# mhauskn/dqn-hfo

Hardware: AMD Instinct MI355X
Metric: DQN updates/sec, 1v0 HFO, 4x1024 MLP, minibatch 256 (higher is better)
Workload: dtype f32

## Files before the change

dqn-hfo_amd/capi.py:

```python
import ctypes as C
import os

from ._build import LIB, build

MAX_HIDDEN = 8
NSTEP_MAX = 64
DP_ID_BYTES = 128
DP_PER_LAYER, DP_HALF_GRADS, DP_SHARD_OPT = 1, 2, 4
DP_UNVERIFIED_OK = 256
TUNE_FP16_WGRAD_PER_LAYER = 1
TUNE_SEPARATE_HEAD_SEED = 2
TUNE_BWD_UNSHIFTED = 4
TUNE_SEPARATE_ACTOR_HEAD_BWD = 8
TUNE_SEPARATE_Q_TRAIN = 16
TUNE_SEPARATE_FIRST_LAYER = 32
TUNE_SEPARATE_CRITIC_FIRST_LAYERS = 64
TUNE_LATE_GATHER = 128
TUNE_NO_KERNARG_PRELOAD = 256
PLAN_FORMS = ("fp16", "data_parallel", "bwd_shifted_critic", "bwd_shifted_actor", "head_wgrad_rides_critic", "head_wgrad_rides_actor",
              "q_train_in_dgrad", "head_seed_fused", "dqda_head_bwd", "critic_l0_rides", "first_layers_merged", "early_gather_l0", "dp_tails_ride", "prioritized", "n_step", "target_smoothing")
LOSS_SCALE_STATIC, LOSS_SCALE_DYNAMIC = 0, 1
FP32, FP16 = 0, 1
ACTOR, CRITIC, ACTOR_TARGET, CRITIC_TARGET = 0, 1, 2, 3
KIND_W, KIND_M, KIND_V, KIND_G = 0, 1, 2, 3
SOLVERS = ("Adam", "SGD", "Nesterov", "AdaGrad", "RMSProp", "AdaDelta")


LR_POLICIES = ("fixed", "step", "exp", "inv", "multistep", "poly", "sigmoid")
LR_MAX_STEPVALUES = 16
REGULARIZATIONS = ("L2", "L1")


class Config(C.Structure):
# ... 282 lines not shown
```

dqn-hfo_amd/csrc/gemm_bodies.hip.h:

```cpp
#pragma once
#include <hip/hip_runtime.h>

#include <cstdint>

#include "learner_args.hip.h"

namespace dqnhip {


__host__ __device__ __forceinline__ void tile_of_counts(int tiles_p, int tiles_q, int b, int& tile_p, int& tile_q) {
  const bool xmap = (tiles_p & 7) == 0;
  const int j = xmap ? b >> 3 : b;
  const int d = j / tiles_q;
  tile_q = j - d * tiles_q;
  tile_p = xmap ? d * 8 + (b & 7) : d;
}
constexpr int kTileDecodeMaxQ = 1024, kTileDecodeMaxTiles = 1 << 18;
__host__ __device__ __forceinline__ uint32_t tile_magic(int tiles_q) { return (uint32_t)((0x80000000ull + (uint32_t)tiles_q - 1) / (uint32_t)tiles_q); }
__host__ __device__ __forceinline__ bool tile_magic_covers(int tiles_p, int tiles_q) {
  return tiles_p >= 1 && tiles_q >= 1 && tiles_q <= kTileDecodeMaxQ && (int64_t)tiles_p * tiles_q <= kTileDecodeMaxTiles;
}
__host__ __device__ __forceinline__ void tile_decode(int tiles_p, int tiles_q, uint32_t magic, int b, int& tile_p, int& tile_q) {
  const bool xmap = (tiles_p & 7) == 0;
  const int j = xmap ? b >> 3 : b;
// ... 476 lines not shown
  __syncthreads();
  f32x4 v = f32x4{0.f, 0.f, 0.f, 0.f};
  if (wave == 0) v = reduce_accumulator<1>(smem, 0, lane);
  return v;
}
__device__ __forceinline__ void dgrad_narrow_body(const GemmProblem& pr, int tile_p, int tile_q, float* smem) {
  const f32x4 v = dgrad_narrow_tile<4>(pr, tile_p, tile_q, smem);
  if ((threadIdx.x >> 6) == 0) {
    const int lane = threadIdx.x & 63, li = lane & 15, lg = lane >> 4;
    const int q = tile_q * 16 + li, p = tile_p * 16 + (lg << 2);
    *reinterpret_cast<f32x4*>(pr.C + (size_t)q * pr.ldc + p) = v;
  }
}

constexpr int kWgradRing = 4;
template <int TPB, int TQB>
__device__ __forceinline__ void wgrad_direct_body(const GemmProblem& pr, int tile_p, int tile_q, float* smem) {
  constexpr int NACC = TPB * 4 * TQB * 4;
  const int lane = threadIdx.x & 63, wave = threadIdx.x >> 6;
  const int li = lane & 15, lg = lane >> 4;
  const int p0 = tile_p * 64 * TPB, q0 = tile_q * 64 * TQB;
  const int Kw = pr.Kred >> 2;
  const int nst = Kw >> 2;
  const int wave_u = __builtin_amdgcn_readfirstlane(wave);
  const char* pp = reinterpret_cast<const char*>(pr.P + (size_t)(wave_u * Kw) * pr.ldp + p0);
  const char* qp = reinterpret_cast<const char*>(pr.Q + (size_t)(wave_u * Kw) * pr.ldq + q0);
  const uint32_t lofp = ((uint32_t)lg * (uint32_t)pr.ldp + (uint32_t)li * 4u) * 4u, lofq = ((uint32_t)lg * (uint32_t)pr.ldq + (uint32_t)li * 4u) * 4u;
  const size_t ldp = (size_t)pr.ldp * 4, ldq = (size_t)pr.ldq * 4;
  const bool want_db = (pr.db != nullptr) && (tile_p == 0);

  f32x4 acc[NACC];
#pragma unroll
  for (int e = 0; e < NACC; ++e) acc[e] = f32x4{0.f, 0.f, 0.f, 0.f};
  f32x4 dbacc[TQB];
#pragma unroll
  for (int d = 0; d < TQB; ++d) dbacc[d] = f32x4{0.f, 0.f, 0.f, 0.f};
  constexpr int NS = kWgradRing;
  f32x4 rp[NS][TPB], rq[NS][TQB];

#define WG_LOAD(slot, st)                                                               \
  {                                                                                     \
    _Pragma("unroll") for (int b = 0; b < TPB; ++b)                                     \
        rp[slot][b] = *reinterpret_cast<const f32x4*>(pp + (size_t)((st) << 2) * ldp + b * 256 + lofp); \
    _Pragma("unroll") for (int d = 0; d < TQB; ++d)                                     \
        rq[slot][d] = *reinterpret_cast<const f32x4*>(qp + (size_t)((st) << 2) * ldq + d * 256 + lofq); \
  }
#define WG_COMPUTE(slot)                                                                \
  {                                                                                     \
    _Pragma("unroll") for (int d = 0; d < TQB; ++d) {                                   \
      dbacc[d].x += rq[slot][d].x; dbacc[d].y += rq[slot][d].y;                         \
      dbacc[d].z += rq[slot][d].z; dbacc[d].w += rq[slot][d].w;                         \
      _Pragma("unroll") for (int qc = 0; qc < 4; ++qc)                                  \
// ... 6 lines not shown

  const int nstN = nst - nst % NS;
  if (nstN > 0) {
#pragma unroll
    for (int i = 0; i < NS; ++i) { WG_LOAD(i, i) DQN_PIN(); }
    int st = 0;
    for (; st + NS < nstN; st += NS) {
#pragma unroll
      for (int i = 0; i < NS; ++i) { WG_COMPUTE(i) DQN_PIN(); WG_LOAD(i, st + NS + i) DQN_PIN(); }
    }
#pragma unroll
    for (int i = 0; i < NS; ++i) { WG_COMPUTE(i) }
  }
  {
    const int rem = nst - nstN;
    if (rem > 0) WG_LOAD(0, nstN)
    if (rem > 1) WG_LOAD(1, nstN + 1)
    if (rem > 2) WG_LOAD(2, nstN + 2)
    if (rem > 0) WG_COMPUTE(0)
    if (rem > 1) WG_COMPUTE(1)
    if (rem > 2) WG_COMPUTE(2)
  }
#undef WG_LOAD
#undef WG_COMPUTE

  park_accumulators<NACC>(smem, acc, wave, lane);
  float* sdb = smem + 4 * NACC * 64 * 4;
  if (want_db) {
#pragma unroll
    for (int d = 0; d < TQB; ++d) {
      f32x4 v = dbacc[d];
      v.x += __shfl_xor(v.x, 16, 64); v.y += __shfl_xor(v.y, 16, 64); v.z += __shfl_xor(v.z, 16, 64); v.w += __shfl_xor(v.w, 16, 64);
      v.x += __shfl_xor(v.x, 32, 64); v.y += __shfl_xor(v.y, 32, 64); v.z += __shfl_xor(v.z, 32, 64); v.w += __shfl_xor(v.w, 32, 64);
      if (lg == 0) reinterpret_cast<f32x4*>(sdb)[(wave * TQB + d) * 16 + li] = v;
    }
  }
  __syncthreads();
  float ssq = 0.0f;
#pragma unroll
  for (int g4 = 0; g4 < TQB * 4 * TPB; ++g4) {
    if ((g4 & 3) == wave) {
      const int b = g4 % TPB, dq = g4 / TPB, qc = dq & 3, d = dq >> 2;
      f32x4 r0 = reduce_accumulator<NACC>(smem, g4 * 4 + 0, lane);
      f32x4 r1 = reduce_accumulator<NACC>(smem, g4 * 4 + 1, lane);
      f32x4 r2 = reduce_accumulator<NACC>(smem, g4 * 4 + 2, lane);
      f32x4 r3 = reduce_accumulator<NACC>(smem, g4 * 4 + 3, lane);
      const int n = q0 + d * 64 + (li << 2) + qc;
#pragma unroll
      for (int r = 0; r < 4; ++r) {
        const int p = p0 + b * 64 + (lg << 4) + (r << 2);
        const f32x4 v = f32x4{r0[r], r1[r], r2[r], r3[r]};
        ssq = fmaf(v.x, v.x, ssq); ssq = fmaf(v.y, v.y, ssq); ssq = fmaf(v.z, v.z, ssq); ssq = fmaf(v.w, v.w, ssq);
        *reinterpret_cast<f32x4*>(pr.C + (size_t)n * pr.ldc + p) = v;
      }
    }
  }
  if (want_db && wave == 0 && lane < 16 * TQB) {
    const int d = lane >> 4, l16 = lane & 15;
    const f32x4* s4 = reinterpret_cast<const f32x4*>(sdb);
    const f32x4 a0 = s4[(0 * TQB + d) * 16 + l16], a1 = s4[(1 * TQB + d) * 16 + l16];
    const f32x4 a2 = s4[(2 * TQB + d) * 16 + l16], a3 = s4[(3 * TQB + d) * 16 + l16];
    f32x4 v;
    v.x = (a0.x + a1.x) + (a2.x + a3.x); v.y = (a0.y + a1.y) + (a2.y + a3.y);
    v.z = (a0.z + a1.z) + (a2.z + a3.z); v.w = (a0.w + a1.w) + (a2.w + a3.w);
    *reinterpret_cast<f32x4*>(pr.db + q0 + d * 64 + (l16 << 2)) = v;
    ssq = fmaf(v.x, v.x, ssq); ssq = fmaf(v.y, v.y, ssq); ssq = fmaf(v.z, v.z, ssq); ssq = fmaf(v.w, v.w, ssq);
  }
  if (pr.partial != nullptr) {
    ssq = wave_sum64(ssq);
    __syncthreads();
    if (lane == 0) smem[wave] = ssq;
    __syncthreads();
    if (threadIdx.x == 0) pr.partial[tile_q * pr.tiles_p + tile_p] = (smem[0] + smem[1]) + (smem[2] + smem[3]);
  }
}

template <int TPB>
__device__ __forceinline__ void wgrad_narrow_body(const GemmProblem& pr, int tile_p, int tile_q, float* smem) {
  constexpr int NACC = TPB * 4;
  const int lane = threadIdx.x & 63, wave = threadIdx.x >> 6;
  const int li = lane & 15, lg = lane >> 4;
  const int p0 = tile_p * 64 * TPB, q0 = tile_q * 16;
  const int Kw = pr.Kred >> 2;
  const int nst = Kw >> 2;
  const int wave_u = __builtin_amdgcn_readfirstlane(wave);
  const char* pp = reinterpret_cast<const char*>(pr.P + (size_t)(wave_u * Kw) * pr.ldp + p0);
  const char* qp = reinterpret_cast<const char*>(pr.Q + (size_t)(wave_u * Kw) * pr.ldq + q0);
  const uint32_t lofp = ((uint32_t)lg * (uint32_t)pr.ldp + (uint32_t)li * 4u) * 4u, lofq = ((uint32_t)lg * (uint32_t)pr.ldq + (uint32_t)li) * 4u;
// ... 453 lines not shown
```

dqn-hfo_amd/csrc/gemm_common.hip.h:

```cpp
#pragma once
#include <hip/hip_runtime.h>
#include <hip/hip_ext.h>
#include <stdint.h>

namespace dqnhip {

typedef float f32x4 __attribute__((ext_vector_type(4)));

enum GemmMode { GEMM_FWD = 0, GEMM_DGRAD = 1, GEMM_WGRAD = 2 };

constexpr float kLeakySlope = 0.01f;

struct GemmProblem {
  const float* P; int ldp;
  const float* Q; int ldq;
  float* C; int ldc;
  int Pdim, Qdim, Kred;
  const float* bias;
  const float* mask; int ldm;
  float* db;
  float* partial;
  int relu;
  const float* seed_w; float* C2;
  const float* dot_w; float* dot_out;
// ... 1 lines not shown
  int mode;
  int tiles_p, tiles_q, tile_base;
};

constexpr int kMaxLeadingDim = 1 << 26;
constexpr int kMaxGroup = 4;
struct GemmBatch {
  GemmProblem prob[kMaxGroup];
  int n;
  int total_tiles;
};

struct alignas(64) GemmHeader {
  int tile_base[kMaxGroup];
  int tiles_p[kMaxGroup], tiles_q[kMaxGroup];
  int n, total_tiles, pad[2];
};
struct alignas(64) GemmHot {
  const float* P; const float* Q;
  int ldp, ldq, Kred, ldc;
  float* C;
  int mode;
  int Pdim, Qdim;
  uint32_t tq_magic;
  int pad[2];
};
struct GemmCold {
  const float* bias; const float* mask; float* db; float* partial;
  const float* seed_w; float* C2; const float* dot_w; float* dot_out; float* xcopy_dst;
  int ldm, relu, xcopy_col, xcopy_n;
};
// ... 13 lines not shown
  uint32_t flags;
};
static_assert(sizeof(GemmPreload) == 14 * 4, "16 user SGPRs less the kernarg pointer");
constexpr uint32_t kPreValid = 1;
constexpr int kPreSplitShift = 2, kPreTilesQShift = 20;
constexpr uint32_t kPreNoSplit = (1u << (32 - kPreSplitShift)) - 1;
#define DQN_PRELOAD_PARAMS const float* pre_P0, const float* pre_Q0, const float* pre_P1, const float* pre_Q1, \
    uint32_t pre_ldp, uint32_t pre_ldq, uint32_t pre_Kred, uint32_t pre_tiles, uint32_t pre_magic, uint32_t pre_flags
#define DQN_PRELOAD_WORDS(pre) (pre).P0, (pre).Q0, (pre).P1, (pre).Q1, (pre).ldp, (pre).ldq, (pre).Kred, (pre).tiles, (pre).magic, (pre).flags
#define DQN_PRELOAD_BLOCK GemmPreload{pre_P0, pre_Q0, pre_P1, pre_Q1, pre_ldp, pre_ldq, pre_Kred, pre_tiles, pre_magic, pre_flags}

struct LaunchOn {
  hipStream_t stream;
  hipEvent_t start = nullptr, stop = nullptr;
  bool no_preload = false;
  LaunchOn(hipStream_t s) : stream(s) {}
  LaunchOn(hipStream_t s, hipEvent_t t0, hipEvent_t t1) : stream(s), start(t0), stop(t1) {}
};
template <typename K, typename... A>
inline hipError_t launch(const LaunchOn& on, K kernel, dim3 grid, dim3 block, size_t lds, const A&... args) {
  if (on.start) hipExtLaunchKernelGGL(kernel, grid, block, (uint32_t)lds, on.stream, on.start, on.stop, 0, args...);
  else hipLaunchKernelGGL(kernel, grid, block, lds, on.stream, args...);
  return hipGetLastError();
}

__device__ __forceinline__ float lrelu_fwd(float x) {
  return fmaxf(x, 0.0f) + kLeakySlope * fminf(x, 0.0f);
}
__device__ __forceinline__ float lrelu_mask(float y) {
  return (y > 0.0f ? 1.0f : 0.0f) + kLeakySlope * (y <= 0.0f ? 1.0f : 0.0f);
// ... 45 lines not shown
```

dqn-hfo_amd/csrc/gemm_direct.hip.h:

```cpp
#pragma once
#include <hip/hip_runtime.h>

#include <algorithm>
#include <cstdint>
#include <cstdlib>

#include "gemm_bodies.hip.h"
#include "gemm_plan.hip.h"

namespace dqnhip {

template <int TP, int TQ>
__global__ __launch_bounds__(256) void gemm_fwd_direct(const GemmArgs<kMaxGroup> args) {
  extern __shared__ __attribute__((aligned(16))) float smem[];
  int tile_p, tile_q;
  const GemmProblem pr = problem_of_block(args, tile_p, tile_q);
  fwd_direct_body<TP, TQ>(pr, tile_p, tile_q, smem);
}
template <int TP, int TQ, bool PIN, int NSLOT = 2>
__global__ __launch_bounds__(256) void gemm_fwd_lds(DQN_PRELOAD_PARAMS, const GemmArgs<kMaxGroup> args) {
  extern __shared__ __attribute__((aligned(16))) float smem[];
  int tile_p, tile_q;
  if (!(pre_flags & kPreValid)) {
    const GemmProblem pr = problem_of_block(args, tile_p, tile_q);
// ... 60 lines not shown
}
template <int TQD = 1, bool DLDS = false>
__global__ __launch_bounds__(256) void gemm_bwd_pair_direct(const GemmArgs<kMaxGroup> args) {
  extern __shared__ __attribute__((aligned(16))) float smem[];
  int tile_p, tile_q;
  const GemmProblem pr = problem_of_block(args, tile_p, tile_q);
  if (pr.mode == GEMM_WGRAD) wgrad_direct_body<1, 1>(pr, tile_p, tile_q, smem);
  else if constexpr (DLDS) dgrad_lds_body<1, TQD, false>(pr, tile_p, tile_q, smem);
  else dgrad_direct_body<1, TQD>(pr, tile_p, tile_q, smem);
}

template <bool DLDS>
__device__ __forceinline__ void bwd_seq_block(const GemmArgs<2>& args, const int block, float* smem) {
  int tile_p, tile_q;
  HotArgs<2> r;
  const int b = request_args(args, r, block);
  const GemmProblem pw = problem_at<1>(args, r);
  if (b < pw.tiles_p * pw.tiles_q) {
    tile_of_record<1>(r, b, tile_p, tile_q);
    wgrad_direct_body<1, 1>(pw, tile_p, tile_q, smem);
  }
  __syncthreads();
  const GemmProblem pd = problem_at<0>(args, r);
  if (b < pd.tiles_p * pd.tiles_q) {
    tile_of_record<0>(r, b, tile_p, tile_q);
    if constexpr (DLDS) dgrad_lds_body<1, 1, true>(pd, tile_p, tile_q, smem);
    else dgrad_direct_body<1, 1>(pd, tile_p, tile_q, smem);
  }
}
template <bool DLDS>
__global__ __launch_bounds__(256) void gemm_bwd_seq(const GemmArgs<2> args) {
// ... 26 lines not shown
  HotArgs<2> r;
  int blk = request_args(args, r, (int)blockIdx.x, tails.on, rider.blocks);
  int tile_p, tile_q;
  if (tails.on && blk == tails.on - 1) { tails_block(tails, smem, reinterpret_cast<double*>(smem + 8)); return; }
  if (blk < rider.blocks) { head_wgrad_rider<NH>(rider, blk, smem); return; }
  blk -= rider.blocks;
  const int n0 = r.hd.tiles_p[1] * r.hd.tiles_q[1];
  if (blk < n0) { const GemmProblem p0 = problem_at<1>(args, r); tile_of_record<1>(r, blk, tile_p, tile_q); wgrad_narrow_body<1>(p0, tile_p, tile_q, smem); return; }
  blk -= n0;
  const GemmProblem p1 = problem_at<0>(args, r);
  tile_of_record<0>(r, blk, tile_p, tile_q); wgrad_direct_body<1, 1>(p1, tile_p, tile_q, smem);
}


constexpr int kBwdTileLds = 4 * 16 * 64 * 16 + 4 * 16 * 16;
constexpr int kWgradTailLdsMax = 80 * 1024;

inline int tile_batch(GemmBatch& batch, int BP, int BQ) {
  int base = 0;
  for (int i = 0; i < batch.n; ++i) {
    GemmProblem& p = batch.prob[i];
    p.tiles_p = p.Pdim / BP;
    p.tiles_q = p.Qdim / BQ;
    p.tile_base = base;
    base += p.tiles_p * p.tiles_q;
  }
  return batch.total_tiles = base;
}
template <typename K>
inline hipError_t direct_launch(K kernel, GemmBatch& batch, int BP, int BQ, int lds_bytes, const LaunchOn& on) {
// ... 118 lines not shown
  w1.tiles_p = w1.Pdim / 64; w1.tiles_q = w1.Qdim / 64; w1.tile_base = 0;
  w0.tiles_p = w0.Pdim / 64; w0.tiles_q = w0.Qdim / 16; w0.tile_base = w1.tiles_p * w1.tiles_q;
  const int grid = w0.tile_base + w0.tiles_p * w0.tiles_q + rider.blocks + (tails.on ? 1 : 0);
  batch.total_tiles = grid;
  if (tails.on) tails.on = grid;
  const size_t lds = std::max(rider.blocks ? head_rider_lds_bytes<NH>(rider) : (size_t)0, (size_t)kBwdTileLds);
  if (lds > (size_t)kWgradTailLdsMax) return hipErrorInvalidValue;
  GemmArgs<2> args;
  if (batch.n != 2 || !pack_args(batch, args)) return hipErrorInvalidValue;
  const GemmPreload pre = make_preload_record(args, 0, on.no_preload, rider.blocks + w0.tiles_p * w0.tiles_q);
  return launch(on, gemm_wgrad_tail<NH>, dim3(grid), dim3(256), lds, DQN_PRELOAD_WORDS(pre), args, rider, tails);
}
template <bool DLDS>
inline hipError_t bwd_seq_launch(GemmBatch& batch, const LaunchOn& on) {
  GemmProblem& d = batch.prob[0]; GemmProblem& w = batch.prob[1];
  d.tiles_p = d.Pdim / 64; d.tiles_q = d.Qdim / 16; d.tile_base = 0;
  w.tiles_p = w.Pdim / 64; w.tiles_q = w.Qdim / 64; w.tile_base = 0;
  const int nd = d.tiles_p * d.tiles_q, nw = w.tiles_p * w.tiles_q;
  const int grid = nd > nw ? nd : nw;
  batch.total_tiles = grid;
  GemmArgs<2> args;
  if (batch.n != 2 || !pack_args(batch, args, false)) return hipErrorInvalidValue;
  return launch(on, gemm_bwd_seq<DLDS>, dim3(grid), dim3(256), kBwdTileLds, args);
}
template <int UNUSED = 0>
inline hipError_t gemm_form_launch(int form, GemmBatch& b, const LaunchOn& on, const HeadWgradRider* rider = nullptr, const TailsArgs* tails = nullptr) {
  if (!gemm_form_accepts(form, b)) return hipErrorInvalidValue;
  const bool tail = form == GEMM_FORM_WGRAD_TAIL_1 || form == GEMM_FORM_WGRAD_TAIL_NO;
  if (!tail && (rider != nullptr || tails != nullptr)) return hipErrorInvalidValue;
  const HeadWgradRider no_rider{};
// ... 11 lines not shown
    case GEMM_FORM_BWD_SEQ: return bwd_seq_launch<false>(b, on);
    case GEMM_FORM_BWD_SEQ_LDS: return bwd_seq_launch<true>(b, on);
    case GEMM_FORM_BWD_PAIR: return bwd_pair_direct_launch<1, false>(b, on);
    case GEMM_FORM_BWD_PAIR_LDS: return bwd_pair_direct_launch<1, true>(b, on);
    case GEMM_FORM_WGRAD_TAIL_1: return wgrad_tail_launch<1>(b, rider ? *rider : no_rider, on, tails);
    case GEMM_FORM_WGRAD_TAIL_NO: return wgrad_tail_launch<kNO>(b, rider ? *rider : no_rider, on, tails);
  }
  return hipErrorInvalidValue;
}
template <typename K>
inline hipError_t direct_prepare(K kernel, int lds_bytes) {
  return hipFuncSetAttribute(reinterpret_cast<const void*>(kernel), hipFuncAttributeMaxDynamicSharedMemorySize, lds_bytes);
}
template <int UNUSED = 0>
inline hipError_t direct_prepare_all() {
  hipError_t e = direct_prepare(gemm_bwd_seq<true>, kBwdTileLds);
  if (e == hipSuccess) e = direct_prepare(gemm_bwd_seq<false>, kBwdTileLds);
  if (e == hipSuccess) e = direct_prepare(gemm_wgrad_tail<1>, kWgradTailLdsMax);
  if (e == hipSuccess) e = direct_prepare(gemm_wgrad_tail<10>, kWgradTailLdsMax);
  if (e == hipSuccess) e = direct_prepare(gemm_bwd_pair_direct<1, true>, kBwdTileLds);
  if (e == hipSuccess) e = direct_prepare(gemm_bwd_pair_direct<1, false>, kBwdTileLds);
  if (e == hipSuccess) e = direct_prepare(gemm_fwd_lds<4, 2, true>, fwd_lds_bytes<4, 2, true>());
  return e;
}

}
```

dqn-hfo_amd/csrc/gemm_plan.hip.h:

```cpp
#pragma once
#include "gemm_common.hip.h"

namespace dqnhip {

enum GemmForm {
  GEMM_FORM_FWD_DIRECT_2x2 = 0, GEMM_FORM_FWD_DIRECT_4x2 = 1,
  GEMM_FORM_FWD_LDS_1x1 = 2, GEMM_FORM_FWD_LDS_2x2 = 3, GEMM_FORM_FWD_LDS_4x2 = 4, GEMM_FORM_FWD_LDS_4x2_ONE_IMAGE = 5,
  GEMM_FORM_DGRAD_DIRECT = 6, GEMM_FORM_DGRAD_LDS = 7, GEMM_FORM_DGRAD_NARROW = 8, GEMM_FORM_WGRAD_NARROW = 9,
  GEMM_FORM_BWD_SEQ = 10, GEMM_FORM_BWD_SEQ_LDS = 11,
  GEMM_FORM_BWD_PAIR = 12, GEMM_FORM_BWD_PAIR_LDS = 13,
  GEMM_FORM_WGRAD_TAIL_1 = 14, GEMM_FORM_WGRAD_TAIL_NO = 15,
  GEMM_FORM_COUNT = 16
};
enum GemmFormKind { GEMM_KIND_FWD_DIRECT, GEMM_KIND_FWD_LDS, GEMM_KIND_DGRAD, GEMM_KIND_DGRAD_NARROW, GEMM_KIND_WGRAD_NARROW,
                    GEMM_KIND_BWD , GEMM_KIND_TAIL };
struct GemmFormSpec { GemmFormKind kind; int bp, bq; bool lds; int n_min, n_max; const char* name; };
inline constexpr GemmFormSpec kGemmForms[GEMM_FORM_COUNT] = {
    {GEMM_KIND_FWD_DIRECT, 32, 32, false, 1, kMaxGroup, "fwd_direct<2,2>"},
    {GEMM_KIND_FWD_DIRECT, 64, 32, false, 1, kMaxGroup, "fwd_direct<4,2>"},
    {GEMM_KIND_FWD_LDS, 16, 16, true, 1, kMaxGroup, "fwd_lds<1,1,true>"},
    {GEMM_KIND_FWD_LDS, 32, 32, true, 1, kMaxGroup, "fwd_lds<2,2,true>"},
    {GEMM_KIND_FWD_LDS, 64, 32, true, 1, kMaxGroup, "fwd_lds<4,2,true>"},
    {GEMM_KIND_FWD_LDS, 64, 32, true, 1, kMaxGroup, "fwd_lds<4,2,true,1>"},
    {GEMM_KIND_DGRAD, 64, 16, false, 1, kMaxGroup, "dgrad_direct<1,1>"},
// ... 39 lines not shown
    case GEMM_KIND_FWD_DIRECT: case GEMM_KIND_FWD_LDS:
      for (int i = 0; i < b.n; ++i) if (!gemm_fwd_accepts(b.prob[i], f)) return false;
      return true;
    case GEMM_KIND_DGRAD: case GEMM_KIND_DGRAD_NARROW:
      for (int i = 0; i < b.n; ++i) if (!gemm_dgrad_accepts(b.prob[i], f.lds, f.kind == GEMM_KIND_DGRAD_NARROW)) return false;
      return true;
    case GEMM_KIND_WGRAD_NARROW:
      for (int i = 0; i < b.n; ++i) if (!gemm_wgrad_accepts(b.prob[i], true)) return false;
      return true;
    case GEMM_KIND_BWD: return gemm_dgrad_accepts(b.prob[0], f.lds, false) && gemm_wgrad_accepts(b.prob[1], false);
    case GEMM_KIND_TAIL: return gemm_wgrad_accepts(b.prob[0], false) && gemm_wgrad_accepts(b.prob[1], true);
  }
  return false;
}

inline GemmForm fwd_form(int kred, int pdim, int rows, int n) {
  const bool lds = gemm_lds_ok(kred);
  if (n == 1) {
    if (lds && rows <= 128) return GEMM_FORM_FWD_LDS_1x1;
    if (lds && rows >= 512 && pdim % 64 == 0) return GEMM_FORM_FWD_LDS_4x2;
    return lds ? GEMM_FORM_FWD_LDS_2x2 : GEMM_FORM_FWD_DIRECT_2x2;
  }
  const long t42 = (long)n * (pdim / 64) * (rows / 32), t22 = (long)n * (pdim / 32) * (rows / 32);
  if (lds) {
    if (t42 >= 192) return GEMM_FORM_FWD_LDS_4x2_ONE_IMAGE;
    if (t22 >= 128 || rows > 128 || rows % 16) return GEMM_FORM_FWD_LDS_2x2;
    return GEMM_FORM_FWD_LDS_1x1;
  }
  return t42 >= 64 ? GEMM_FORM_FWD_DIRECT_4x2 : GEMM_FORM_FWD_DIRECT_2x2;
}
// ... 19 lines not shown
```

dqn-hfo_amd/csrc/learner.hip:

```cpp
#include "learner_internal.hip.h"
#include "gemm_direct.hip.h"
#include "hgemm.hip.h"
#include "head_fwd_kernels.hip.h"
#include "head_kernels.hip.h"
#include "small_kernels.hip.h"
#include "solver_kernels.hip.h"

using namespace dqnhip;
using namespace dqnhip_host;

namespace dqnhip_host {

const char* const kFamily[kNumFamily] = {"gemm_fwd_lds_4x2", "gemm_dgrad", "gemm_wgrad", "adam", "gemm_bwd_pair", "gemm_fwd_lds_2x2", "gemm_fwd_direct",
                                         "hgemm_fwd", "hgemm_dgrad", "hgemm_wgrad",
                                         "per_sync", "per_sample", "per_update"};
static Family family_of(GemmForm f, int n) {
  switch (kGemmForms[f].kind) {
    case GEMM_KIND_FWD_DIRECT: return kFamFwdDirect;
    case GEMM_KIND_FWD_LDS: return n == 1 ? kFamFwdLds2x2 : kFamFwdLds4x2;
    case GEMM_KIND_DGRAD: case GEMM_KIND_DGRAD_NARROW: return kFamDgrad;
    case GEMM_KIND_BWD: return kFamBwdPair;
    case GEMM_KIND_WGRAD_NARROW: case GEMM_KIND_TAIL: break;
  }
  return kFamWgrad;
}
static int form_check(GemmForm f, const GemmBatch& b) {
  return gemm_form_accepts(f, b) ? 0 : fail("internal: the carrier %s of a rider does not accept its problems", kGemmForms[f].name);
}
static int form_launch(H* h, hipStream_t st, GemmForm f, GemmBatch& b, const HeadWgradRider* rider = nullptr, const TailsArgs* tails = nullptr) {
  HIPCHK(gemm_form_launch(f, b, timed(h, family_of(f, b.n), st), rider, tails));
  return 0;
}


int layer_forward(H* h, hipStream_t st, const FwdPass* passes, int n, int rows, int i) {
  const NetLayout& l = *passes[0].l;
  GemmBatch b{}; b.n = n;
  for (int j = 0; j < n; ++j) {
    GemmProblem& p = b.prob[j];
    p.P = wat(h, passes[j].net, l.w_off[i]); p.ldp = l.kp[i];
    p.Q = passes[j].act[i]; p.ldq = l.kp[i];
    p.C = passes[j].act[i + 1]; p.ldc = l.kp[i + 1];
    p.Pdim = l.dims[i + 1]; p.Qdim = rows; p.Kred = l.kp[i];
    p.bias = wat(h, passes[j].net, l.b_off[i]); p.relu = 1;
    if (i == l.L - 1 && passes[j].seed_w != nullptr) { p.seed_w = passes[j].seed_w; p.C2 = passes[j].seed_out; }
// ... 836 lines not shown
```

dqn-hfo_amd/csrc/learner_internal.hip.h:

```cpp
#pragma once
#include <hip/hip_runtime.h>
#include <rccl/rccl.h>
#include <zlib.h>
#include <unistd.h>

#include <algorithm>
#include <cmath>
#include <cstdarg>
#include <cstdio>
#include <cstdlib>
#include <cstring>
#include <deque>
#include <random>
#include <string>
#include <vector>
#include <mutex>
#include <chrono>
#include <thread>

#include "../../include/dqnhip.h"
#include "../../include/dqnhip_env.h"
#include "gemm_common.hip.h"
#include "learner_args.hip.h"
#include "noise_bodies.hip.h"
// ... 181 lines not shown
  unsigned long long chain_epoch = 0, chain_ring_epoch = 0;
  std::vector<int32_t> chain_idx;
  int* idx_next_pinned[2] = {nullptr, nullptr}; const int* idx_next_dev[2] = {nullptr, nullptr};
  hipEvent_t pipe_ev[2] = {nullptr, nullptr};
  int* pipe_idx_dev[2] = {nullptr, nullptr}; int* pipe_idx_pinned[2] = {nullptr, nullptr};
  float* pipe_stats[2] = {nullptr, nullptr};
  unsigned long long pipe_count = 0;
  int* ix_idx[kIxBanks] = {nullptr}; const int* ix_idx_dev[kIxBanks] = {nullptr};
  float* ix_stats[kIxBanks] = {nullptr}; float* ix_stats_dev[kIxBanks] = {nullptr};
  hipEvent_t ix_ev[kIxBanks] = {nullptr};
  int ix_busy[kIxBanks] = {0};
  int ix_next = 0;
  hipGraphExec_t ix_graph[kIxBanks][kIxSizes] = {{nullptr}};
  long long opt_launches[3] = {0, 0, 0};
  LrSchedule sched{}; LrSchedule* sched_dev = nullptr;
  long long sched_launches[2] = {0, 0};
  int ix_nodes[kIxSizes] = {0};
  const int* cap_idx = nullptr;
  float* cap_stats = nullptr;
  std::deque<float> ix_pairs;
  std::deque<std::pair<unsigned long long, int>> ix_flagged;
  unsigned long long ix_harvested = 0, ix_collected = 0;
  int ix_prev_flags = 0;
  long long per_env_slack = 0;
  PerHost* per = nullptr;
  TargetNoiseHost* tnoise = nullptr;
  NstepHost* nstep = nullptr;
  DiagHost* diag = nullptr;
  SweepHost* sweep = nullptr;
  hipGraphExec_t sweep_graph[2] = {nullptr, nullptr};
// ... 15 lines not shown
  RingUse(H* h) : o(RO(h)), st(h->stream), on(RO(h)->ring_shared) {
    if (!on) return;
    o->ring_mu.lock();
    if (o->ring_ev_valid && o->ring_last != st) hipStreamWaitEvent(st, o->ring_ev, 0);
  }
  ~RingUse() {
    if (!on) return;
    hipEventRecord(o->ring_ev, st); o->ring_last = st; o->ring_ev_valid = true;
    o->ring_mu.unlock();
  }
};

inline LaunchOn timed(H* h, Family fam, hipStream_t st) {
  LaunchOn on(st);
  on.no_preload = (h->cfg.tuning_flags & DQNHIP_TUNE_NO_KERNARG_PRELOAD) != 0;
  if (!h->timing) return on;
  hipEventCreate(&on.start); hipEventCreate(&on.stop);
  h->recs.push_back({fam, on.start, on.stop});
  return on;
}

void dense_to_arena(const NetLayout& l, const float* dense, std::vector<float>& arena);
void arena_to_dense(const NetLayout& l, const std::vector<float>& arena, float* dense);
inline const NetLayout& layout_of(const H* h, int net) { return (net & 1) ? h->lc : h->la; }
int validate(const dqnhip_config* c, dqnhip_config* full);
LrSchedule schedule_of(const dqnhip_config& c);
inline bool has_policy(const H* h) { return h->cfg.lr_policy != DQNHIP_LR_FIXED; }
inline bool has_decay(const H* h) { return h->cfg.weight_decay != 0.0f; }
inline bool sched_family(const H* h) { return has_decay(h) || (has_policy(h) && h->cfg.solver_type != DQNHIP_SOLVER_ADAM); }
inline bool dp_exchanges(const H* h) { return h->cfg.dp_world > 1 || h->dp_half || h->dp_shard; }
// ... 106 lines not shown
```

dqn-hfo_amd/csrc/learner_io.hip:

```cpp
#include "learner_internal.hip.h"
#include "head_fwd_kernels.hip.h"
#include "io_kernels.hip.h"

namespace dqnhip_host {

static int pack_blocks16(int rows, int k16) { return (rows * ((k16 + 511) / 512) + 3) / 4; }
int pack_rows16_launch(hipStream_t st, const float* src, int n, int S, int ld_src, h16* dst, int rows, int k16) {
  HIPCHK(launch(st, k_pack_rows16, dim3(pack_blocks16(rows, k16)), dim3(256), 0, Pack16Args{src, nullptr, n, S, ld_src, dst, rows, k16}));
  return 0;
}
bool same_nets(const H* a, const H* b) {
  if (a->S != b->S || a->L != b->L) return false;
  for (int i = 0; i < a->L; ++i) if (a->cfg.hidden[i] != b->cfg.hidden[i]) return false;
  return true;
}

}

extern "C" {


static int actor_forward16_dev(H* h, int net, const float* states_dev, int n, float* out_dev) {
  const int rows = act16_rows(n);
  RC(ensure_act16(h, rows));
// ... 563 lines not shown
int dqnhip_debug_read(dqnhip_handle h, const char* name, float* host, size_t count) {
  if (!h || !name || !host) return fail("null argument");
  HIPCHK(hipSetDevice(h->cfg.device));
  const size_t B = h->B;
  const float* src = nullptr; size_t n = B; bool pad16 = false; bool is_int = false;
  if (!strcmp(name, "optimiser_launches")) {
    if (count < 3) return fail("buffer too small for '%s'", name);
    for (int k = 0; k < 3; ++k) host[k] = (float)h->opt_launches[k];
    return 0;
  }
  if (!strcmp(name, "sched_launches")) {
    if (count < 2) return fail("buffer too small for '%s'", name);
    for (int k = 0; k < 2; ++k) host[k] = (float)h->sched_launches[k];
    return 0;
  }
  if (!strcmp(name, "indexed_graph_launches")) {
    if (count < 1) return fail("buffer too small for '%s'", name);
    for (size_t k = 0; k < std::min(count, (size_t)kIxSizes); ++k) host[k] = (float)h->ix_nodes[k];
    return 0;
  }
  if (!strcmp(name, "q_target")) src = h->q_t;
  else if (!strcmp(name, "y")) src = h->y;
  else if (!strcmp(name, "q_train")) src = h->q1;
  else if (!strcmp(name, "q_policy")) src = h->q2;
  else if (!strcmp(name, "terminal")) src = h->mb_term;
  else if (!strcmp(name, "actor_out")) { src = h->aout16; pad16 = true; n = B * kNO; }
  else if (!strcmp(name, "dq_da")) { src = h->dA16; pad16 = true; n = B * kNO; }
  else if (!strcmp(name, "idx")) { src = (const float*)h->mb_idx; is_int = true; }
  else if (!strncmp(name, "act", 3) && name[3] >= '0' && name[3] <= '4' && name[4] == '_') {
    const int p = name[3] - '0', i = atoi(name + 5);
// ... 111 lines not shown
```

dqn-hfo_amd/learner.py:

```python
import ctypes as C
import os
from collections import namedtuple

import numpy as np

from . import capi
from .capi import ACTOR, CRITIC, ACTOR_TARGET, CRITIC_TARGET, KIND_W, KIND_M, KIND_V, KIND_G

kActionSize = 4
kActionParamSize = 6
kStateInputCount = 1
DASH, TURN, TACKLE, KICK = 0, 1, 2, 3

Action = namedtuple("Action", "action arg1 arg2")
Transition = namedtuple("Transition", "state actor_output reward on_policy_target next_state")


class DQNFatal(RuntimeError):
    """The reference's CHECK/LOG(FATAL) abort, as an exception."""


def _f32(a):
    return np.ascontiguousarray(a, dtype=np.float32)

# ... 564 lines not shown
            self._ck(self.lib.dqnhip_debug_read(self.h, name.encode(), _p(out), out.size))
            return out
        if name in ("dz_c", "dz_a"):
            width = self.cfg.hidden[self.cfg.num_hidden - 1]
            out = np.empty(B * width, np.float32)
            self._ck(self.lib.dqnhip_debug_read(self.h, name.encode(), _p(out), out.size))
            return out.reshape(B, width)
        if name == "optimiser_launches":
            out = np.zeros(3, np.float32)
            self._ck(self.lib.dqnhip_debug_read(self.h, name.encode(), _p(out), out.size))
            return out.astype(np.int64)
        if name == "sched_launches":
            out = np.zeros(2, np.float32)
            self._ck(self.lib.dqnhip_debug_read(self.h, name.encode(), _p(out), out.size))
            return out.astype(np.int64)
        wide = name in ("actor_out", "dq_da", "actor_target_out", "dxc", "actor_target_smoothed", "target_noise_z")
        out = np.empty(B * (10 if wide else 1), np.float32)
        self._ck(self.lib.dqnhip_debug_read(self.h, name.encode(), _p(out), out.size))
        return out.reshape(B, 10) if wide else out

    def grad_buffer(self, net):
        ptr, n = C.c_void_p(), C.c_size_t()
        self._ck(self.lib.dqnhip_grad_buffer(self.h, net, C.byref(ptr), C.byref(n)))
        return ptr.value, n.value

    def stream(self):
        s = C.c_void_p()
        self._ck(self.lib.dqnhip_get_stream(self.h, C.byref(s)))
        return s.value

# ... 417 lines not shown
```

include/dqnhip.h:

```cpp
#ifndef DQNHIP_H_
#define DQNHIP_H_

#include <stddef.h>
#include <stdint.h>

#ifdef __cplusplus
extern "C" {
#endif

#define DQNHIP_ACTION_SIZE 4
#define DQNHIP_ACTION_PARAM_SIZE 6
#define DQNHIP_ACTOR_OUT 10
#define DQNHIP_MAX_HIDDEN 8

enum dqnhip_net {
  DQNHIP_ACTOR = 0,
  DQNHIP_CRITIC = 1,
  DQNHIP_ACTOR_TARGET = 2,
  DQNHIP_CRITIC_TARGET = 3
};

enum dqnhip_param_kind {
  DQNHIP_KIND_W = 0,
  DQNHIP_KIND_M = 1,
// ... 68 lines not shown
  int32_t loss_scale_mode;
  int32_t loss_scale_growth_interval;
  float loss_scale_min_mult;
  float loss_scale_max_mult;
} dqnhip_config;

#define DQNHIP_TUNE_FP16_WGRAD_PER_LAYER 1
#define DQNHIP_TUNE_SEPARATE_HEAD_SEED 2
#define DQNHIP_TUNE_BWD_UNSHIFTED 4
#define DQNHIP_TUNE_SEPARATE_ACTOR_HEAD_BWD 8
#define DQNHIP_TUNE_SEPARATE_Q_TRAIN 16
#define DQNHIP_TUNE_SEPARATE_FIRST_LAYER 32
#define DQNHIP_TUNE_SEPARATE_CRITIC_FIRST_LAYERS 64
#define DQNHIP_TUNE_LATE_GATHER 128
#define DQNHIP_TUNE_NO_KERNARG_PRELOAD 256

typedef struct dqnhip_learner* dqnhip_handle;

void dqnhip_default_config(dqnhip_config* cfg, int32_t state_size);

const char* dqnhip_solver_name(int32_t solver_type);
const char* dqnhip_lr_policy_name(int32_t lr_policy);

size_t dqnhip_grad_arena_bytes(const dqnhip_config* cfg);

const char* dqnhip_last_error(void);

int dqnhip_create(const dqnhip_config* cfg, dqnhip_handle* out);
int dqnhip_destroy(dqnhip_handle h);

// ... 317 lines not shown
```

Before: 3758.

## Use wider tiles and interleaved roles in the LDS backward-sequential kernel

Adds a 'wide' mode for the fused dgrad+wgrad backward kernel. Dgrad tiles become 64x32 and wgrad tiles 64x128 with an 8-deep load ring, which cuts the block count and increases operand reuse per block. The first blocks interleave dgrad and wgrad roles in groups of eight so both kinds of work are spread across the GPU. The wide path needs more LDS and more registers per block, which may lower occupancy. The clip-norm partials become per 64-column sub-tile, and a tuning flag can turn the wide path off.

```diff
diff --git a/dqn-hfo_amd/capi.py b/dqn-hfo_amd/capi.py
--- a/dqn-hfo_amd/capi.py
+++ b/dqn-hfo_amd/capi.py
@@ -17,6 +17,7 @@
 TUNE_SEPARATE_CRITIC_FIRST_LAYERS = 64
 TUNE_LATE_GATHER = 128
 TUNE_NO_KERNARG_PRELOAD = 256
+TUNE_BWD_SEQ_NARROW = 512
 PLAN_FORMS = ("fp16", "data_parallel", "bwd_shifted_critic", "bwd_shifted_actor", "head_wgrad_rides_critic", "head_wgrad_rides_actor",
               "q_train_in_dgrad", "head_seed_fused", "dqda_head_bwd", "critic_l0_rides", "first_layers_merged", "early_gather_l0", "dp_tails_ride", "prioritized", "n_step", "target_smoothing")
 LOSS_SCALE_STATIC, LOSS_SCALE_DYNAMIC = 0, 1
diff --git a/dqn-hfo_amd/csrc/gemm_bodies.hip.h b/dqn-hfo_amd/csrc/gemm_bodies.hip.h
--- a/dqn-hfo_amd/csrc/gemm_bodies.hip.h
+++ b/dqn-hfo_amd/csrc/gemm_bodies.hip.h
@@ -514,7 +514,7 @@
 }
 
 constexpr int kWgradRing = 4;
-template <int TPB, int TQB>
+template <int TPB, int TQB, int NS = kWgradRing>
 __device__ __forceinline__ void wgrad_direct_body(const GemmProblem& pr, int tile_p, int tile_q, float* smem) {
   constexpr int NACC = TPB * 4 * TQB * 4;
   const int lane = threadIdx.x & 63, wave = threadIdx.x >> 6;
@@ -535,7 +535,6 @@
   f32x4 dbacc[TQB];
 #pragma unroll
   for (int d = 0; d < TQB; ++d) dbacc[d] = f32x4{0.f, 0.f, 0.f, 0.f};
-  constexpr int NS = kWgradRing;
   f32x4 rp[NS][TPB], rq[NS][TQB];
 
 #define WG_LOAD(slot, st)                                                               \
@@ -572,12 +571,10 @@
   }
   {
     const int rem = nst - nstN;
-    if (rem > 0) WG_LOAD(0, nstN)
-    if (rem > 1) WG_LOAD(1, nstN + 1)
-    if (rem > 2) WG_LOAD(2, nstN + 2)
-    if (rem > 0) WG_COMPUTE(0)
-    if (rem > 1) WG_COMPUTE(1)
-    if (rem > 2) WG_COMPUTE(2)
+#pragma unroll
+    for (int i = 0; i < NS - 1; ++i) if (rem > i) WG_LOAD(i, nstN + i)
+#pragma unroll
+    for (int i = 0; i < NS - 1; ++i) if (rem > i) WG_COMPUTE(i)
   }
 #undef WG_LOAD
 #undef WG_COMPUTE
@@ -594,7 +591,9 @@
     }
   }
   __syncthreads();
-  float ssq = 0.0f;
+  float ssq[TQB];
+#pragma unroll
+  for (int d = 0; d < TQB; ++d) ssq[d] = 0.0f;
 #pragma unroll
   for (int g4 = 0; g4 < TQB * 4 * TPB; ++g4) {
     if ((g4 & 3) == wave) {
@@ -608,28 +607,37 @@
       for (int r = 0; r < 4; ++r) {
         const int p = p0 + b * 64 + (lg << 4) + (r << 2);
         const f32x4 v = f32x4{r0[r], r1[r], r2[r], r3[r]};
-        ssq = fmaf(v.x, v.x, ssq); ssq = fmaf(v.y, v.y, ssq); ssq = fmaf(v.z, v.z, ssq); ssq = fmaf(v.w, v.w, ssq);
+        ssq[d] = fmaf(v.x, v.x, ssq[d]); ssq[d] = fmaf(v.y, v.y, ssq[d]); ssq[d] = fmaf(v.z, v.z, ssq[d]); ssq[d] = fmaf(v.w, v.w, ssq[d]);
         *reinterpret_cast<f32x4*>(pr.C + (size_t)n * pr.ldc + p) = v;
       }
     }
   }
-  if (want_db && wave == 0 && lane < 16 * TQB) {
-    const int d = lane >> 4, l16 = lane & 15;
+  if (want_db && wave == 0 && lane < 16) {
     const f32x4* s4 = reinterpret_cast<const f32x4*>(sdb);
-    const f32x4 a0 = s4[(0 * TQB + d) * 16 + l16], a1 = s4[(1 * TQB + d) * 16 + l16];
-    const f32x4 a2 = s4[(2 * TQB + d) * 16 + l16], a3 = s4[(3 * TQB + d) * 16 + l16];
-    f32x4 v;
-    v.x = (a0.x + a1.x) + (a2.x + a3.x); v.y = (a0.y + a1.y) + (a2.y + a3.y);
-    v.z = (a0.z + a1.z) + (a2.z + a3.z); v.w = (a0.w + a1.w) + (a2.w + a3.w);
-    *reinterpret_cast<f32x4*>(pr.db + q0 + d * 64 + (l16 << 2)) = v;
-    ssq = fmaf(v.x, v.x, ssq); ssq = fmaf(v.y, v.y, ssq); ssq = fmaf(v.z, v.z, ssq); ssq = fmaf(v.w, v.w, ssq);
+#pragma unroll
+    for (int d = 0; d < TQB; ++d) {
+      const f32x4 a0 = s4[(0 * TQB + d) * 16 + lane], a1 = s4[(1 * TQB + d) * 16 + lane];
+      const f32x4 a2 = s4[(2 * TQB + d) * 16 + lane], a3 = s4[(3 * TQB + d) * 16 + lane];
+      f32x4 v;
+      v.x = (a0.x + a1.x) + (a2.x + a3.x); v.y = (a0.y + a1.y) + (a2.y + a3.y);
+      v.z = (a0.z + a1.z) + (a2.z + a3.z); v.w = (a0.w + a1.w) + (a2.w + a3.w);
+      *reinterpret_cast<f32x4*>(pr.db + q0 + d * 64 + (lane << 2)) = v;
+      ssq[d] = fmaf(v.x, v.x, ssq[d]); ssq[d] = fmaf(v.y, v.y, ssq[d]); ssq[d] = fmaf(v.z, v.z, ssq[d]); ssq[d] = fmaf(v.w, v.w, ssq[d]);
+    }
   }
   if (pr.partial != nullptr) {
-    ssq = wave_sum64(ssq);
+#pragma unroll
+    for (int d = 0; d < TQB; ++d) ssq[d] = wave_sum64(ssq[d]);
     __syncthreads();
-    if (lane == 0) smem[wave] = ssq;
+    if (lane == 0) {
+#pragma unroll
+      for (int d = 0; d < TQB; ++d) smem[d * 4 + wave] = ssq[d];
+    }
     __syncthreads();
-    if (threadIdx.x == 0) pr.partial[tile_q * pr.tiles_p + tile_p] = (smem[0] + smem[1]) + (smem[2] + smem[3]);
+    if ((int)threadIdx.x < TQB) {
+      const int d = threadIdx.x;
+      pr.partial[(tile_q * TQB + d) * pr.tiles_p + tile_p] = (smem[d * 4 + 0] + smem[d * 4 + 1]) + (smem[d * 4 + 2] + smem[d * 4 + 3]);
+    }
   }
 }
 
diff --git a/dqn-hfo_amd/csrc/gemm_common.hip.h b/dqn-hfo_amd/csrc/gemm_common.hip.h
--- a/dqn-hfo_amd/csrc/gemm_common.hip.h
+++ b/dqn-hfo_amd/csrc/gemm_common.hip.h
@@ -39,7 +39,9 @@
 struct alignas(64) GemmHeader {
   int tile_base[kMaxGroup];
   int tiles_p[kMaxGroup], tiles_q[kMaxGroup];
-  int n, total_tiles, pad[2];
+  int n, total_tiles;
+  int wide;
+  int pad;
 };
 struct alignas(64) GemmHot {
   const float* P; const float* Q;
@@ -83,6 +85,7 @@
   hipStream_t stream;
   hipEvent_t start = nullptr, stop = nullptr;
   bool no_preload = false;
+  bool no_wide = false;
   LaunchOn(hipStream_t s) : stream(s) {}
   LaunchOn(hipStream_t s, hipEvent_t t0, hipEvent_t t1) : stream(s), start(t0), stop(t1) {}
 };
diff --git a/dqn-hfo_amd/csrc/gemm_direct.hip.h b/dqn-hfo_amd/csrc/gemm_direct.hip.h
--- a/dqn-hfo_amd/csrc/gemm_direct.hip.h
+++ b/dqn-hfo_amd/csrc/gemm_direct.hip.h
@@ -98,7 +98,22 @@
 __device__ __forceinline__ void bwd_seq_block(const GemmArgs<2>& args, const int block, float* smem) {
   int tile_p, tile_q;
   HotArgs<2> r;
-  const int b = request_args(args, r, block);
+  const int b = request_args(args, r, block, args.head.wide);
+  if constexpr (DLDS) {
+    if (r.hd.wide != 0) {
+      const WideRole role = bwd_wide_role((r.hd.wide - 1) >> 1, r.hd.tiles_p[1] * r.hd.tiles_q[1], b);
+      if (role.wgrad) {
+        const GemmProblem pw = problem_at<1>(args, r);
+        tile_of_record<1>(r, role.tile, tile_p, tile_q);
+        wgrad_direct_body<1, kWideWgradQ / 64, kWideWgradRing>(pw, tile_p, tile_q, smem);
+      } else {
+        const GemmProblem pd = problem_at<0>(args, r);
+        tile_of_record<0>(r, role.tile, tile_p, tile_q);
+        dgrad_lds_body<1, kWideDgradQ / 16, true>(pd, tile_p, tile_q, smem);
+      }
+      return;
+    }
+  }
   const GemmProblem pw = problem_at<1>(args, r);
   if (b < pw.tiles_p * pw.tiles_q) {
     tile_of_record<1>(r, b, tile_p, tile_q);
@@ -155,6 +170,7 @@
 
 
 constexpr int kBwdTileLds = 4 * 16 * 64 * 16 + 4 * 16 * 16;
+constexpr int kBwdWideLds = 4 * (kWideWgradQ / 64) * 16 * 64 * 16 + 4 * (kWideWgradQ / 64) * 16 * 16;
 constexpr int kWgradTailLdsMax = 80 * 1024;
 
 inline int tile_batch(GemmBatch& batch, int BP, int BQ) {
@@ -303,6 +319,16 @@
 template <bool DLDS>
 inline hipError_t bwd_seq_launch(GemmBatch& batch, const LaunchOn& on) {
   GemmProblem& d = batch.prob[0]; GemmProblem& w = batch.prob[1];
+  if (DLDS && bwd_wide_accepts(GEMM_FORM_BWD_SEQ_LDS, batch, on.no_wide)) {
+    d.tiles_p = d.Pdim / kWideDgradP; d.tiles_q = d.Qdim / kWideDgradQ; d.tile_base = 0;
+    w.tiles_p = w.Pdim / kWideWgradP; w.tiles_q = w.Qdim / kWideWgradQ; w.tile_base = 0;
+    const int nd = d.tiles_p * d.tiles_q, nw = w.tiles_p * w.tiles_q;
+    batch.total_tiles = nd + nw;
+    GemmArgs<2> args;
+    if (!pack_args(batch, args, false)) return hipErrorInvalidValue;
+    args.head.wide = 2 * bwd_wide_inter(nw, nd) + 1;
+    return launch(on, gemm_bwd_seq<DLDS>, dim3(nd + nw), dim3(256), kBwdWideLds, args);
+  }
   d.tiles_p = d.Pdim / 64; d.tiles_q = d.Qdim / 16; d.tile_base = 0;
   w.tiles_p = w.Pdim / 64; w.tiles_q = w.Qdim / 64; w.tile_base = 0;
   const int nd = d.tiles_p * d.tiles_q, nw = w.tiles_p * w.tiles_q;
@@ -344,7 +370,7 @@
 }
 template <int UNUSED = 0>
 inline hipError_t direct_prepare_all() {
-  hipError_t e = direct_prepare(gemm_bwd_seq<true>, kBwdTileLds);
+  hipError_t e = direct_prepare(gemm_bwd_seq<true>, kBwdWideLds);
   if (e == hipSuccess) e = direct_prepare(gemm_bwd_seq<false>, kBwdTileLds);
   if (e == hipSuccess) e = direct_prepare(gemm_wgrad_tail<1>, kWgradTailLdsMax);
   if (e == hipSuccess) e = direct_prepare(gemm_wgrad_tail<10>, kWgradTailLdsMax);
diff --git a/dqn-hfo_amd/csrc/gemm_plan.hip.h b/dqn-hfo_amd/csrc/gemm_plan.hip.h
--- a/dqn-hfo_amd/csrc/gemm_plan.hip.h
+++ b/dqn-hfo_amd/csrc/gemm_plan.hip.h
@@ -77,6 +77,31 @@
   return false;
 }
 
+constexpr int kWideDgradP = 64, kWideDgradQ = 32, kWideWgradP = 64, kWideWgradQ = 128;
+constexpr int kWideMaxTiles = 256;
+constexpr int kWideWgradRing = 8;
+inline bool bwd_wide_dims_ok(int d_pdim, int d_qdim, int d_kred, int w_pdim, int w_qdim, int w_kred) {
+  if (d_pdim <= 0 || d_qdim <= 0 || w_pdim <= 0 || w_qdim <= 0) return false;
+  if (d_pdim % kWideDgradP || d_qdim % kWideDgradQ || w_pdim % kWideWgradP || w_qdim % kWideWgradQ) return false;
+  if ((long)(d_pdim / kWideDgradP) * (d_qdim / kWideDgradQ) + (long)(w_pdim / kWideWgradP) * (w_qdim / kWideWgradQ) > kWideMaxTiles) return false;
+  return gemm_lds_ok(d_kred) && w_kred >= 4 * 4 * kWideWgradRing && w_kred % (4 * 4 * kWideWgradRing) == 0;
+}
+inline bool bwd_wide_accepts(int form, const GemmBatch& b, bool no_wide = false) {
+  if (no_wide || form != GEMM_FORM_BWD_SEQ_LDS || !gemm_form_accepts(form, b)) return false;
+  const GemmProblem &d = b.prob[0], &w = b.prob[1];
+  return bwd_wide_dims_ok(d.Pdim, d.Qdim, d.Kred, w.Pdim, w.Qdim, w.Kred);
+}
+struct WideRole { bool wgrad; int tile; };
+__host__ __device__ __forceinline__ int bwd_wide_inter(int n_wgrad, int n_dgrad) { return (n_wgrad < n_dgrad ? n_wgrad : n_dgrad) & ~7; }
+__host__ __device__ __forceinline__ WideRole bwd_wide_role(int inter, int n_wgrad, int b) {
+  WideRole r;
+  if (b < 2 * inter) { r.wgrad = !((b >> 3) & 1); r.tile = ((b >> 4) << 3) | (b & 7); return r; }
+  const int x = b - 2 * inter, left = n_wgrad - inter;
+  r.wgrad = x < left;
+  r.tile = inter + (r.wgrad ? x : x - left);
+  return r;
+}
+
 inline GemmForm fwd_form(int kred, int pdim, int rows, int n) {
   const bool lds = gemm_lds_ok(kred);
   if (n == 1) {
diff --git a/dqn-hfo_amd/csrc/learner.hip b/dqn-hfo_amd/csrc/learner.hip
--- a/dqn-hfo_amd/csrc/learner.hip
+++ b/dqn-hfo_amd/csrc/learner.hip
@@ -28,7 +28,9 @@
   return gemm_form_accepts(f, b) ? 0 : fail("internal: the carrier %s of a rider does not accept its problems", kGemmForms[f].name);
 }
 static int form_launch(H* h, hipStream_t st, GemmForm f, GemmBatch& b, const HeadWgradRider* rider = nullptr, const TailsArgs* tails = nullptr) {
-  HIPCHK(gemm_form_launch(f, b, timed(h, family_of(f, b.n), st), rider, tails));
+  const LaunchOn on = timed(h, family_of(f, b.n), st);
+  if (bwd_wide_accepts(f, b, on.no_wide)) h->bwd_wide_launches += 1;
+  HIPCHK(gemm_form_launch(f, b, on, rider, tails));
   return 0;
 }
 
diff --git a/dqn-hfo_amd/csrc/learner_internal.hip.h b/dqn-hfo_amd/csrc/learner_internal.hip.h
--- a/dqn-hfo_amd/csrc/learner_internal.hip.h
+++ b/dqn-hfo_amd/csrc/learner_internal.hip.h
@@ -219,6 +219,7 @@
   hipGraphExec_t ix_graph[kIxBanks][kIxSizes] = {{nullptr}};
   long long opt_launches[3] = {0, 0, 0};
   LrSchedule sched{}; LrSchedule* sched_dev = nullptr;
+  long long bwd_wide_launches = 0;
   long long sched_launches[2] = {0, 0};
   int ix_nodes[kIxSizes] = {0};
   const int* cap_idx = nullptr;
@@ -264,6 +265,7 @@
 inline LaunchOn timed(H* h, Family fam, hipStream_t st) {
   LaunchOn on(st);
   on.no_preload = (h->cfg.tuning_flags & DQNHIP_TUNE_NO_KERNARG_PRELOAD) != 0;
+  on.no_wide = (h->cfg.tuning_flags & DQNHIP_TUNE_BWD_SEQ_NARROW) != 0;
   if (!h->timing) return on;
   hipEventCreate(&on.start); hipEventCreate(&on.stop);
   h->recs.push_back({fam, on.start, on.stop});
diff --git a/dqn-hfo_amd/csrc/learner_io.hip b/dqn-hfo_amd/csrc/learner_io.hip
--- a/dqn-hfo_amd/csrc/learner_io.hip
+++ b/dqn-hfo_amd/csrc/learner_io.hip
@@ -601,6 +601,20 @@
     for (int k = 0; k < 2; ++k) host[k] = (float)h->sched_launches[k];
     return 0;
   }
+  if (!strcmp(name, "bwd_wide_launches")) {
+    if (count < 1) return fail("buffer too small for '%s'", name);
+    host[0] = (float)h->bwd_wide_launches;
+    return 0;
+  }
+  if (!strcmp(name, "clip_partials_a") || !strcmp(name, "clip_partials_c")) {
+    const int net = name[14] == 'c';
+    const size_t np = (size_t)layout_of(h, net).n_part;
+    if (count < np + 1) return fail("buffer too small for '%s': %zu < %zu", name, count, np + 1);
+    HIPCHK(hipStreamSynchronize(h->stream));
+    HIPCHK(hipMemcpy(host + 1, h->part[net], np * sizeof(float), hipMemcpyDeviceToHost));
+    host[0] = (float)np;
+    return 0;
+  }
   if (!strcmp(name, "indexed_graph_launches")) {
     if (count < 1) return fail("buffer too small for '%s'", name);
     for (size_t k = 0; k < std::min(count, (size_t)kIxSizes); ++k) host[k] = (float)h->ix_nodes[k];
diff --git a/dqn-hfo_amd/learner.py b/dqn-hfo_amd/learner.py
--- a/dqn-hfo_amd/learner.py
+++ b/dqn-hfo_amd/learner.py
@@ -602,6 +602,14 @@
             out = np.zeros(2, np.float32)
             self._ck(self.lib.dqnhip_debug_read(self.h, name.encode(), _p(out), out.size))
             return out.astype(np.int64)
+        if name == "bwd_wide_launches":
+            out = np.zeros(1, np.float32)
+            self._ck(self.lib.dqnhip_debug_read(self.h, name.encode(), _p(out), out.size))
+            return int(out[0])
+        if name in ("clip_partials_a", "clip_partials_c"):
+            out = np.zeros(1 + self.param_count(int(name[-1] == "c")), np.float32)
+            self._ck(self.lib.dqnhip_debug_read(self.h, name.encode(), _p(out), out.size))
+            return out[1:1 + int(out[0])].copy()
         wide = name in ("actor_out", "dq_da", "actor_target_out", "dxc", "actor_target_smoothed", "target_noise_z")
         out = np.empty(B * (10 if wide else 1), np.float32)
         self._ck(self.lib.dqnhip_debug_read(self.h, name.encode(), _p(out), out.size))
diff --git a/include/dqnhip.h b/include/dqnhip.h
--- a/include/dqnhip.h
+++ b/include/dqnhip.h
@@ -106,6 +106,7 @@
 #define DQNHIP_TUNE_SEPARATE_CRITIC_FIRST_LAYERS 64
 #define DQNHIP_TUNE_LATE_GATHER 128
 #define DQNHIP_TUNE_NO_KERNARG_PRELOAD 256
+#define DQNHIP_TUNE_BWD_SEQ_NARROW 512
 
 typedef struct dqnhip_learner* dqnhip_handle;
 
```

New measurement: 3785, median of 6. No clear change (+0.7%).
